# QinLab-WFU/CLIP-based-Cross-Modal-Hashing

Hardware: AMD Instinct MI355X
Metric: image+text pairs/s encoded+hashed per GPU; mAP@K eval wallclock (64-bit) (higher is better)
Workload: dtype bf16

## Files before the change

clip-based-cross-modal-hashing_amd/csrc/gemm_lc.hip:

```cpp
#include <cstdlib>
#include <cstring>

#include "cmh_common.h"

#include <hip/hip_ext.h>

namespace cmh {

typedef __attribute__((ext_vector_type(8))) __bf16 lc_bf16x8_t;
typedef __attribute__((ext_vector_type(4))) float lc_f32x4_t;
typedef __attribute__((ext_vector_type(2))) float lc_f32x2_t;
typedef __attribute__((ext_vector_type(4))) uint32_t lc_u32x4_t;
typedef __attribute__((ext_vector_type(2))) unsigned lc_u2_t;
typedef const __attribute__((address_space(1))) void* lc_gptr_t;
typedef __attribute__((address_space(3))) void* lc_lptr_t;

constexpr int lcBM = 128, lcBN = 256;
constexpr int lcRowBytes = 128;
constexpr int lcWBytes = lcBN * lcRowBytes;
constexpr int lcSTG = lcWBytes + lcBM * lcRowBytes;

struct LcProblem {
  const char* X; const char* W; const float* bias; const void* residual; void* out;
  const int* m_dev;
  int Mub, N, K;
  const float* colscale = nullptr;
  float alpha = 1.f, oscale = 1.f;
};

__device__ __forceinline__ int lc_swz(int row, int chunk) { return row * lcRowBytes + ((chunk ^ (row & 7)) << 4); }

#define LC_READ(dst, addr, off) asm volatile("ds_read_b128 %0, %1 offset:" #off : "=v"(dst) : "v"(addr))
typedef const __attribute__((address_space(3))) lc_u32x4_t* lc_lds_u4p;
__device__ __forceinline__ lc_u32x4_t lc_lds_read(uint32_t addr) { return *reinterpret_cast<lc_lds_u4p>(static_cast<size_t>(addr)); }

#ifdef LC_STAMPS
__device__ unsigned long long g_lc_stamps[256 * 8];
#define LC_T() __builtin_amdgcn_s_memtime()
#endif


template <int BM, bool GRP, int BK = 64>
struct LcSchedule {
  int M0, M1;
  int tiles_n0, tiles_n1, slot, per;
  DealShare sh0, sh1;
  int n_first, my_tiles;
  int nk0, nk1, S;
  __device__ __forceinline__ LcSchedule(const LcProblem& p0, const LcProblem& p1) {
    M0 = p0.Mub;
    if (p0.m_dev) { const int md = *p0.m_dev; M0 = md < M0 ? md : M0; }
    M0 = __builtin_amdgcn_readfirstlane(M0);
    M1 = 0;
    if constexpr (GRP) {
      M1 = p1.Mub;
      if (p1.m_dev) { const int md = *p1.m_dev; M1 = md < M1 ? md : M1; }
      M1 = __builtin_amdgcn_readfirstlane(M1);
    }
    tiles_n0 = p0.N / lcBN; tiles_n1 = GRP ? p1.N / lcBN : 1;
    const int total0 = tiles_n0 * ((M0 + BM - 1) / BM);
    const int total1 = GRP ? tiles_n1 * ((M1 + BM - 1) / BM) : 0;
    const int xcd = blockIdx.x & 7;
    slot = blockIdx.x >> 3; per = gridDim.x >> 3;
    sh0 = deal_share(total0, xcd); sh1 = deal_share(total1, xcd);
    n_first = deal_count(sh0.len, slot, per);
    my_tiles = deal_count(sh0.len + sh1.len, slot, per);
  }
  __device__ __forceinline__ void count_ksteps(const LcProblem& p0, const LcProblem& p1) {
    nk0 = p0.K / BK; nk1 = GRP ? p1.K / BK : 0;
    S = n_first * nk0 + (my_tiles - n_first) * nk1;
  }
  __device__ void tile_of(int ti, bool& second, int& m0, int& n0) const {
    second = GRP && ti >= n_first;
    const int logical = deal_tile(slot + ti * per, second, sh0, sh1);
    const int tn_cnt = second ? tiles_n1 : tiles_n0;
    const int tm = logical / tn_cnt;
    m0 = tm * BM;
    n0 = (logical - tm * tn_cnt) * lcBN;
  }
};

constexpr int lc_pieces(int bm) { return 8 + bm / 32; }
#define LC_VMCNT(n) asm volatile("s_waitcnt vmcnt(%0)" ::"n"(n) : "memory")
template <int BM, bool GRP, int ABL = 0, int LDS_BYTES>
__device__ __forceinline__ void lc_loader_wave(const LcSchedule<BM, GRP>& sc, char (&lds)[LDS_BYTES], int wid, int lane, int epi,
                                               const char* X0, const char* W0, const float* B0, int K0, const char* X1, const char* W1,
                                               const float* B1, int K1) {
  constexpr int XP = BM / 32;
  constexpr int PIECES = lc_pieces(BM);
  static_assert(2 * PIECES < 64, "the counted waits must fit gfx950's 6-bit vmcnt field");
  constexpr int STG = lcWBytes + BM * lcRowBytes;
  static_assert(LDS_BYTES == 3 * STG + 2 * 1024, "the ring of three stages, then the two bias rows");
  const int sub = lane >> 3, ch = lane & 7;
  uint32_t offW[8], offX[XP];
  const char* Wt = nullptr;
  const char* Xt = nullptr;
  const char* Bt = nullptr;
  int i_nk = 0;
  int w_prob = -1;
  auto set_tile = [&](int ti) {
    bool second; int m0, n0;
    sc.tile_of(ti, second, m0, n0);
    const uint32_t rs = static_cast<uint32_t>(second ? K1 : K0) * 2;
    if (w_prob != static_cast<int>(second)) {
      w_prob = static_cast<int>(second);
#pragma unroll
      for (int i = 0; i < 8; ++i) {
        const int row = (wid * 8 + i) * 8 + sub;
        offW[i] = static_cast<uint32_t>(row) * rs + ((ch ^ (row & 7)) << 4);
      }
    }
    i_nk = second ? sc.nk1 : sc.nk0;
    const int Mp = second ? sc.M1 : sc.M0;
    Wt = (second ? W1 : W0) + static_cast<size_t>(n0) * rs;
    Xt = second ? X1 : X0;
    Bt = reinterpret_cast<const char*>((second ? B1 : B0) + n0);
#pragma unroll
    for (int i = 0; i < XP; ++i) {
      const int row = (wid * XP + i) * 8 + sub;
      int xr = m0 + row;
      xr = xr < Mp ? xr : Mp - 1;
      offX[i] = static_cast<uint32_t>(xr) * rs + ((ch ^ (row & 7)) << 4);
    }
  };
  int i_tile = 0, i_kt = 0, ibuf = 0;
  set_tile(0);
  const bool bias_wave = wid == 0 && (epi & EPI_BIAS);
  auto issue_stage = [&]() {
    char* base = lds + ibuf * STG;
    const uint32_t koff = static_cast<uint32_t>(i_kt) * lcRowBytes;
    if (i_kt == 0 && bias_wave)
      __builtin_amdgcn_global_load_lds((lc_gptr_t)(Bt + lane * 16), (lc_lptr_t)(lds + 3 * STG + (i_tile & 1) * 1024), 16, 0, 0);
#pragma unroll
    for (int i = 0; i < 8; ++i)
      __builtin_amdgcn_global_load_lds((lc_gptr_t)(Wt + koff + offW[i]), (lc_lptr_t)(base + (wid * 8 + i) * 1024), 16, 0, 0);
#pragma unroll
    for (int i = 0; i < XP; ++i)
      __builtin_amdgcn_global_load_lds((lc_gptr_t)(Xt + koff + offX[i]), (lc_lptr_t)(base + lcWBytes + (wid * XP + i) * 1024), 16, 0, 0);
    ibuf = ibuf == 2 ? 0 : ibuf + 1;
    if (++i_kt == i_nk) {
      i_kt = 0;
      if (++i_tile < sc.my_tiles) set_tile(i_tile);
    }
  };
  const int S = sc.S;
  issue_stage();
  if (S > 1) issue_stage();
  if (S > 2) issue_stage();
  if (S > 2) LC_VMCNT(2 * PIECES);
  else if (S > 1) LC_VMCNT(PIECES);
  else LC_VMCNT(0);
  __builtin_amdgcn_s_barrier();
  for (int s = 0; s < S; ++s) {
    if (s + 2 < S && !(ABL & 4)) LC_VMCNT(PIECES);
    else LC_VMCNT(0);
    __builtin_amdgcn_s_barrier();
    if (s + 3 < S && !(ABL & 2)) issue_stage();
  }
}

__device__ __forceinline__ lc_f32x4_t lc_mfma_bf16(const lc_u32x4_t& w, const lc_u32x4_t& x, const lc_f32x4_t& cin) {
  return __builtin_amdgcn_mfma_f32_16x16x32_bf16(__builtin_bit_cast(lc_bf16x8_t, w), __builtin_bit_cast(lc_bf16x8_t, x), cin, 0, 0, 0);
}
template <int NP, int ROW0 = 0>
__device__ __forceinline__ void lc_store_parked(const lc_u32x4_t (&pend)[NP], int idx, char* base, uint32_t off0, uint32_t ldn) {
  static_assert(NP == 4 || NP == 8, "four or eight parked pieces");
  char* p = base + (off0 + static_cast<uint32_t>(ROW0 + (idx >> 1)) * 16u * ldn + static_cast<uint32_t>(idx & 1) * 64u);
  switch (idx) {
    case 0: *reinterpret_cast<lc_u32x4_t*>(p) = pend[0]; break;
    case 1: *reinterpret_cast<lc_u32x4_t*>(p) = pend[1]; break;
    case 2: *reinterpret_cast<lc_u32x4_t*>(p) = pend[2]; break;
    case 3: *reinterpret_cast<lc_u32x4_t*>(p) = pend[3]; break;
    case 4: *reinterpret_cast<lc_u32x4_t*>(p) = pend[NP > 4 ? 4 : 3]; break;
    case 5: *reinterpret_cast<lc_u32x4_t*>(p) = pend[NP > 4 ? 5 : 3]; break;
    case 6: *reinterpret_cast<lc_u32x4_t*>(p) = pend[NP > 4 ? 6 : 3]; break;
    default: *reinterpret_cast<lc_u32x4_t*>(p) = pend[NP - 1]; break;
  }
}
template <int BM, bool GRP>
__device__ __forceinline__ void lc_residual_of(const LcSchedule<BM, GRP>& sc, int ti, int wm, int wn, const void* R0, int N0,
                                               const void* R1, int N1, const uint16_t*& base, int& ld, int& rows) {
  bool second; int m0, n0;
  sc.tile_of(ti, second, m0, n0);
  ld = second ? N1 : N0;
  rows = (second ? sc.M1 : sc.M0) - (m0 + wm * (BM / 2));
  base = reinterpret_cast<const uint16_t*>(second ? R1 : R0) + static_cast<size_t>(m0 + wm * (BM / 2)) * ld + n0 + wn * 64;
}
__device__ __forceinline__ lc_u32x4_t lc_res_piece(const uint16_t* base, int ld, int rows, int frow, int fq, int b, int pr) {
  int r = b * 16 + frow;
  r = r < rows ? r : rows - 1;
  return *reinterpret_cast<const lc_u32x4_t*>(base + static_cast<size_t>(r) * ld + (fq & 1) * 16 + (fq & 2) * 4 + 32 * pr);
// ... 540 lines not shown
constexpr int lc3STG = lcWBytes + lc3BM * lcRowBytes;

template <bool GRP, int RES, bool F16O>
__global__ __launch_bounds__(768) void gemm_lc3_kernel(LcProblem p0, LcProblem p1, int epi) {
  __shared__ __attribute__((aligned(1024))) char lds[3 * lc3STG + 2 * 1024];
  const int tid = threadIdx.x;
  const int lane = tid & 63;
  const int wid = __builtin_amdgcn_readfirstlane(tid >> 6);

  const char* const X0 = p0.X; const char* const W0 = p0.W; const float* const B0 = p0.bias; void* const O0 = p0.out;
  const void* const R0 = p0.residual;
  const int N0 = p0.N, K0 = p0.K;
  const char* const X1 = p1.X; const char* const W1 = p1.W; const float* const B1 = p1.bias; void* const O1 = p1.out;
  const void* const R1 = p1.residual;
  const int N1 = p1.N, K1 = p1.K;
  int M0 = p0.Mub;
  if (p0.m_dev) { const int md = *p0.m_dev; M0 = md < M0 ? md : M0; }
  M0 = __builtin_amdgcn_readfirstlane(M0);
  int M1 = 0;
  if constexpr (GRP) {
    M1 = p1.Mub;
    if (p1.m_dev) { const int md = *p1.m_dev; M1 = md < M1 ? md : M1; }
    M1 = __builtin_amdgcn_readfirstlane(M1);
  }
  const int tiles_n0 = N0 / lcBN, tiles_n1 = GRP ? N1 / lcBN : 1;
  const int total0 = tiles_n0 * ((M0 + lc3BM - 1) / lc3BM);
  const int total1 = GRP ? tiles_n1 * ((M1 + lc3BM - 1) / lc3BM) : 0;
  const int xcd = blockIdx.x & 7, slot = blockIdx.x >> 3, per = gridDim.x >> 3;
  const int q0 = total0 >> 3, r0 = total0 & 7, q1 = total1 >> 3, r1 = total1 & 7;
  const int lo0 = xcd < r0 ? xcd * (q0 + 1) : r0 * (q0 + 1) + (xcd - r0) * q0, len0 = xcd < r0 ? q0 + 1 : q0;
  const int lo1 = xcd < r1 ? xcd * (q1 + 1) : r1 * (q1 + 1) + (xcd - r1) * q1, len1 = xcd < r1 ? q1 + 1 : q1;
  const int n_first = slot < len0 ? (len0 - slot + per - 1) / per : 0;
  const int span = len0 + len1;
  const int my_tiles = slot < span ? (span - slot + per - 1) / per : 0;
  if (my_tiles == 0) return;
  const int nk0 = K0 / 64, nk1 = GRP ? K1 / 64 : 0;
  const int S = n_first * nk0 + (my_tiles - n_first) * nk1;
  auto tile_of = [&](int ti, bool& second, int& m0, int& n0) {
    const int j = slot + ti * per;
    second = GRP && ti >= n_first;
    const int logical = second ? lo1 + (j - len0) : lo0 + j;
    const int tn_cnt = second ? tiles_n1 : tiles_n0;
    const int tm = logical / tn_cnt;
    m0 = tm * lc3BM;
    n0 = (logical - tm * tn_cnt) * lcBN;
  };

  if (wid < 4) {
    const int sub = lane >> 3, ch = lane & 7;
    uint32_t offW[8], offX[5];
    const char* Wt = nullptr;
    const char* Xt = nullptr;
    const char* Bt = nullptr;
    int i_nk = 0;
    int w_prob = -1;
    auto set_tile = [&](int ti) {
      bool second; int m0, n0;
      tile_of(ti, second, m0, n0);
      const uint32_t rs = static_cast<uint32_t>(second ? K1 : K0) * 2;
      if (w_prob != static_cast<int>(second)) {
        w_prob = static_cast<int>(second);
#pragma unroll
        for (int i = 0; i < 8; ++i) {
          const int row = (wid * 8 + i) * 8 + sub;
          offW[i] = static_cast<uint32_t>(row) * rs + ((ch ^ (row & 7)) << 4);
        }
      }
      i_nk = second ? nk1 : nk0;
      const int Mp = second ? M1 : M0;
      Wt = (second ? W1 : W0) + static_cast<size_t>(n0) * rs;
      Xt = second ? X1 : X0;
      Bt = reinterpret_cast<const char*>((second ? B1 : B0) + n0);
#pragma unroll
      for (int i = 0; i < 5; ++i) {
        const int row = (wid * 5 + i) * 8 + sub;
        int xr = m0 + row;
        xr = xr < Mp ? xr : Mp - 1;
        offX[i] = static_cast<uint32_t>(xr) * rs + ((ch ^ (row & 7)) << 4);
      }
    };
    int i_tile = 0, i_kt = 0, ibuf = 0;
    set_tile(0);
    const bool bias_wave = wid == 0 && (epi & EPI_BIAS);
    auto issue_stage = [&]() {
      char* base = lds + ibuf * lc3STG;
      const uint32_t koff = static_cast<uint32_t>(i_kt) * lcRowBytes;
      if (i_kt == 0 && bias_wave)
        __builtin_amdgcn_global_load_lds((lc_gptr_t)(Bt + lane * 16), (lc_lptr_t)(lds + 3 * lc3STG + (i_tile & 1) * 1024), 16, 0, 0);
#pragma unroll
      for (int i = 0; i < 8; ++i)
        __builtin_amdgcn_global_load_lds((lc_gptr_t)(Wt + koff + offW[i]), (lc_lptr_t)(base + (wid * 8 + i) * 1024), 16, 0, 0);
#pragma unroll
      for (int i = 0; i < 5; ++i)
        __builtin_amdgcn_global_load_lds((lc_gptr_t)(Xt + koff + offX[i]), (lc_lptr_t)(base + lcWBytes + (wid * 5 + i) * 1024), 16, 0, 0);
      ibuf = ibuf == 2 ? 0 : ibuf + 1;
      if (++i_kt == i_nk) {
        i_kt = 0;
        if (++i_tile < my_tiles) set_tile(i_tile);
      }
    };
    issue_stage();
    if (S > 1) issue_stage();
    if (S > 2) issue_stage();
    if (S > 2) LC_VMCNT(2 * lc_pieces(lc3BM));
    else if (S > 1) LC_VMCNT(lc_pieces(lc3BM));
    else LC_VMCNT(0);
    __builtin_amdgcn_s_barrier();
    for (int s = 0; s < S; ++s) {
      if (s + 2 < S) LC_VMCNT(lc_pieces(lc3BM));
      else LC_VMCNT(0);
      __builtin_amdgcn_s_barrier();
      if (s + 3 < S) issue_stage();
    }
    return;
  }

  const int c = wid - 4;
  const int wm = c >> 2, wn = c & 3;
  const int frow = lane & 15, fq = lane >> 4;
  const uint32_t lds_base = static_cast<uint32_t>(reinterpret_cast<uintptr_t>((lc_lptr_t)lds));
  const uint32_t aW = lds_base + lc_swz(wn * 64 + frow, fq);
  const uint32_t aX = lds_base + lcWBytes + lc_swz(wm * 80 + frow, fq);

  lc_f32x4_t acc[4][5];
  lc_u32x4_t fw[4], fx[5];
  lc_u32x4_t pend[8];
  int pend_idx = 8;
  char* pend_base = nullptr;
  uint32_t pend_off0 = 0, pend_ldn = 0;
  [[maybe_unused]] int res_kt = -1;
  [[maybe_unused]] const uint16_t* rq_base = nullptr;
  [[maybe_unused]] int rq_ld = 0, rq_rows = 0;

  void* out = O0;
  int N = N0, M = M0, nk = nk0;
  [[maybe_unused]] auto to_problem1 = [&]() { out = O1; N = N1; M = M1; nk = nk1; };
  if constexpr (GRP) { if (n_first == 0) to_problem1(); }

  auto store_pending = [&](int idx) __attribute__((always_inline)) {
    lc_store_parked(pend, idx, pend_base, pend_off0, pend_ldn);
  };
  [[maybe_unused]] auto residual_of = [&](int ti, const uint16_t*& base, int& ld, int& rows) __attribute__((always_inline)) {
    bool second; int m0, n0;
    tile_of(ti, second, m0, n0);
    ld = second ? N1 : N0;
    rows = (second ? M1 : M0) - (m0 + wm * 80);
    base = reinterpret_cast<const uint16_t*>(second ? R1 : R0) + static_cast<size_t>(m0 + wm * 80) * ld + n0 + wn * 64;
  };
  [[maybe_unused]] auto res_piece = [&](const uint16_t* base, int ld, int rows, int b, int pr) __attribute__((always_inline)) {
    return lc_res_piece(base, ld, rows, frow, fq, b, pr);
  };
  [[maybe_unused]] auto add_piece = [&](int b, int pr, const lc_u32x4_t& qv) __attribute__((always_inline)) { lc_add_piece(acc, b, pr, qv); };

  int cur = 0;
  if constexpr (RES == 1) {
    const uint16_t* rb; int ld, rows;
    residual_of(0, rb, ld, rows);
#pragma unroll
    for (int a = 0; a < 4; ++a)
#pragma unroll
      for (int b = 0; b < 5; ++b) acc[a][b] = lc_f32x4_t{0.f, 0.f, 0.f, 0.f};
#pragma unroll
    for (int b = 0; b < 5; ++b)
#pragma unroll
      for (int pr = 0; pr < 2; ++pr) add_piece(b, pr, res_piece(rb, ld, rows, b, pr));
  }
  __builtin_amdgcn_s_barrier();
  asm volatile("" ::: "memory");
#pragma unroll
  for (int b = 0; b < 5; ++b) fx[b] = lc_lds_read(aX + b * 2048);
#pragma unroll
  for (int a = 0; a < 4; ++a) fw[a] = lc_lds_read(aW + a * 2048);

#define L3_GROUP(a)                                                                                    \
  do {                                                                                                 \
    acc[a][0] = lc_mfma_bf16(fw[a], fx[0], acc[a][0]);                                                 \
    acc[a][1] = lc_mfma_bf16(fw[a], fx[1], acc[a][1]);                                                 \
    acc[a][2] = lc_mfma_bf16(fw[a], fx[2], acc[a][2]);                                                 \
    acc[a][3] = lc_mfma_bf16(fw[a], fx[3], acc[a][3]);                                                 \
    acc[a][4] = lc_mfma_bf16(fw[a], fx[4], acc[a][4]);                                                 \
    __builtin_amdgcn_sched_barrier(0);                                                                 \
  } while (0)
#define L3_LAST(wsrc, xsrc)                                                                            \
  do {                                                                                                 \
    acc[3][0] = lc_mfma_bf16(fw[3], fx[0], acc[3][0]);                                                 \
    __builtin_amdgcn_sched_barrier(0);                                                                 \
    fx[0] = lc_lds_read((xsrc));                                                                       \
    __builtin_amdgcn_sched_barrier(0);                                                                 \
    acc[3][1] = lc_mfma_bf16(fw[3], fx[1], acc[3][1]);                                                 \
    __builtin_amdgcn_sched_barrier(0);                                                                 \
    fx[1] = lc_lds_read((xsrc) + 2048);                                                                \
    __builtin_amdgcn_sched_barrier(0);                                                                 \
    acc[3][2] = lc_mfma_bf16(fw[3], fx[2], acc[3][2]);                                                 \
    __builtin_amdgcn_sched_barrier(0);                                                                 \
    fx[2] = lc_lds_read((xsrc) + 4096);                                                                \
    __builtin_amdgcn_sched_barrier(0);                                                                 \
    acc[3][3] = lc_mfma_bf16(fw[3], fx[3], acc[3][3]);                                                 \
    __builtin_amdgcn_sched_barrier(0);                                                                 \
    fx[3] = lc_lds_read((xsrc) + 6144);                                                                \
    __builtin_amdgcn_sched_barrier(0);                                                                 \
    acc[3][4] = lc_mfma_bf16(fw[3], fx[4], acc[3][4]);                                                 \
    __builtin_amdgcn_sched_barrier(0);                                                                 \
    fx[4] = lc_lds_read((xsrc) + 8192);                                                                \
    fw[3] = lc_lds_read((wsrc) + 6144);                                                                \
    __builtin_amdgcn_sched_barrier(0);                                                                 \
  } while (0)
#define L3_REFILL_W(a, wsrc)                                                                           \
  do {                                                                                                 \
    fw[a] = lc_lds_read((wsrc) + (a) * 2048);                                                          \
    __builtin_amdgcn_sched_barrier(0);                                                                 \
  } while (0)

  auto kstep = [&](int kt) __attribute__((always_inline)) {
    const uint32_t bo = static_cast<uint32_t>(cur) * lc3STG;
    const uint32_t w1 = (aW + bo) ^ 64u, x1 = (aX + bo) ^ 64u;
    L3_GROUP(0); L3_REFILL_W(0, w1);
    L3_GROUP(1); L3_REFILL_W(1, w1);
    if (pend_idx < 8) {
      store_pending(pend_idx); store_pending(pend_idx + 1);
      pend_idx += 2;
      asm volatile("" : "+s"(pend_idx));
      __builtin_amdgcn_sched_barrier(0);
    }
    if constexpr (RES != 0) {
      if (kt == res_kt) {
#pragma unroll
        for (int b = 0; b < 4; ++b)
#pragma unroll
          for (int pr = 0; pr < 2; ++pr) pend[2 * b + pr] = res_piece(rq_base, rq_ld, rq_rows, b, pr);
        __builtin_amdgcn_sched_barrier(0);
      }
    }
    L3_GROUP(2); L3_REFILL_W(2, w1);
    L3_LAST(w1, x1);
    const int nxt = cur == 2 ? 0 : cur + 1;
    const uint32_t bn = static_cast<uint32_t>(nxt) * lc3STG;
    const uint32_t w0 = aW + bn, x0 = aX + bn;
    L3_GROUP(0);
    L3_GROUP(1);
    __builtin_amdgcn_s_waitcnt(0xC07F);
    __builtin_amdgcn_s_barrier();
    asm volatile("" ::: "memory");
    __builtin_amdgcn_sched_barrier(0);
    L3_REFILL_W(0, w0); L3_REFILL_W(1, w0);
    L3_GROUP(2); L3_REFILL_W(2, w0);
    L3_LAST(w0, x0);
    cur = nxt;
  };

  for (int ti = 0; ti < my_tiles; ++ti) {
    bool second; int m0, n0;
    tile_of(ti, second, m0, n0);
    if constexpr (GRP) { if (ti == n_first && ti > 0) to_problem1(); }
    if constexpr (RES != 1) {
#pragma unroll
      for (int a = 0; a < 4; ++a)
#pragma unroll
        for (int b = 0; b < 5; ++b) acc[a][b] = lc_f32x4_t{0.f, 0.f, 0.f, 0.f};
    }
    if constexpr (RES == 1) { res_kt = ti + 1 < my_tiles ? 4 : -1; if (ti + 1 < my_tiles) residual_of(ti + 1, rq_base, rq_ld, rq_rows); }
    if constexpr (RES == 2) { res_kt = 4; residual_of(ti, rq_base, rq_ld, rq_rows); }
    if constexpr (RES != 0) asm volatile("" : "+s"(res_kt));
    for (int kt = 0; kt < nk; ++kt) {
      asm volatile("" : "+s"(kt));
      kstep(kt);
    }

    [[maybe_unused]] lc_u32x4_t r4[2];
    if constexpr (RES == 2) { r4[0] = res_piece(rq_base, rq_ld, rq_rows, 4, 0); r4[1] = res_piece(rq_base, rq_ld, rq_rows, 4, 1); }
    if constexpr (RES == 1) {
      if (res_kt >= 0) { r4[0] = res_piece(rq_base, rq_ld, rq_rows, 4, 0); r4[1] = res_piece(rq_base, rq_ld, rq_rows, 4, 1); }
    }
    if (epi & EPI_BIAS) {
      const uint32_t ab = lds_base + 3 * lc3STG + (ti & 1) * 1024 + (wn * 64 + fq * 4) * 4;
      lc_f32x4_t bv[4];
#pragma unroll
      for (int a = 0; a < 4; ++a) bv[a] = __builtin_bit_cast(lc_f32x4_t, lc_lds_read(ab + a * 64));
#pragma unroll
      for (int a = 0; a < 4; ++a)
#pragma unroll
        for (int b = 0; b < 5; ++b) acc[a][b] += bv[a];
    }
    if (epi & EPI_QUICKGELU) lc_quickgelu(acc);
    if constexpr (RES == 2) {
#pragma unroll
      for (int b = 0; b < 4; ++b)
#pragma unroll
        for (int pr = 0; pr < 2; ++pr) add_piece(b, pr, pend[2 * b + pr]);
      add_piece(4, 0, r4[0]); add_piece(4, 1, r4[1]);
    }
    __builtin_amdgcn_sched_barrier(0);
    {
      char* const obase = static_cast<char*>(out) + (static_cast<size_t>(m0) * N + n0) * 2;
      const uint32_t ldn = static_cast<uint32_t>(N) * 2;
      const uint32_t off0 = static_cast<uint32_t>(wm * 80 + frow) * ldn + static_cast<uint32_t>(wn * 64 + (fq & 1) * 16 + (fq & 2) * 4) * 2;
      const bool full = m0 + lc3BM <= M;
      lc_u32x4_t own4[2];
#pragma unroll
      for (int b = 0; b < 5; ++b)
#pragma unroll
        for (int pr = 0; pr < 2; ++pr) {
          const lc_u32x4_t val = lc_pack_piece<F16O>(acc, b, pr);
          if constexpr (RES == 1) {
            const lc_u32x4_t nextres = b < 4 ? pend[2 * b + pr] : r4[pr];
            acc[2 * pr][b] = lc_f32x4_t{0.f, 0.f, 0.f, 0.f};
            acc[2 * pr + 1][b] = lc_f32x4_t{0.f, 0.f, 0.f, 0.f};
            if (res_kt >= 0) add_piece(b, pr, nextres);
          }
          if (b < 4) pend[2 * b + pr] = val;
          else own4[pr] = val;
        }
      if (!(epi & 256)) {
        if (full) {
#pragma unroll
          for (int pr = 0; pr < 2; ++pr) *reinterpret_cast<lc_u32x4_t*>(obase + (off0 + 64u * ldn + pr * 64)) = own4[pr];
        } else if (m0 + wm * 80 + 64 + frow < M) {
#pragma unroll
          for (int pr = 0; pr < 2; ++pr) *reinterpret_cast<lc_u32x4_t*>(obase + (off0 + 64u * ldn + pr * 64)) = own4[pr];
        }
      }
      pend_base = obase; pend_off0 = off0; pend_ldn = ldn;
      if (full && ti + 1 < my_tiles && !(epi & 256)) {
        pend_idx = 0;
        asm volatile("" : "+s"(pend_idx));
      } else if (!(epi & 256)) {
#pragma unroll
        for (int b = 0; b < 4; ++b)
#pragma unroll
          for (int pr = 0; pr < 2; ++pr)
            if (m0 + wm * 80 + b * 16 + frow < M)
              *reinterpret_cast<lc_u32x4_t*>(obase + (off0 + static_cast<uint32_t>(b * 16) * ldn + pr * 64)) = pend[2 * b + pr];
      }
    }
  }
#undef L3_GROUP
#undef L3_LAST
#undef L3_REFILL_W
}

template <bool GRP>
__global__ __launch_bounds__(768) void gemm_lc2q_kernel(LcProblem p0, LcProblem p1, int epi) {
  static_assert(!GRP, "first form: plain launches");
  __shared__ __attribute__((aligned(1024))) char lds[3 * lcSTG];
  const int tid = threadIdx.x;
  const int lane = tid & 63;
  const int wid = __builtin_amdgcn_readfirstlane(tid >> 6);
  const char* const X0 = p0.X; const char* const W0 = p0.W; const float* const B0 = p0.bias; void* const O0 = p0.out;
  const float* const CS0 = p0.colscale; const float alpha0 = p0.alpha;
  const int N0 = p0.N, K0 = p0.K;
  LcSchedule<lcBM, false, 128> sc(p0, p1);
  if (sc.my_tiles == 0) return;
  sc.count_ksteps(p0, p1);
  const int M0 = sc.M0, nk0 = sc.nk0, my_tiles = sc.my_tiles;
  if (wid < 4) {
    const int S = sc.S;
    const int sub = lane >> 3, ch = lane & 7;
    uint32_t offW[8], offX[4];
    const char* Wt = nullptr;
    const uint32_t rs = static_cast<uint32_t>(K0);
#pragma unroll
    for (int i = 0; i < 8; ++i) {
      const int row = (wid * 8 + i) * 8 + sub;
      offW[i] = static_cast<uint32_t>(row) * rs + ((ch ^ (row & 7)) << 4);
    }
    auto set_tile = [&](int ti) {
      bool second; int m0, n0;
      sc.tile_of(ti, second, m0, n0);
      Wt = W0 + static_cast<size_t>(n0) * rs;
#pragma unroll
      for (int i = 0; i < 4; ++i) {
        const int row = (wid * 4 + i) * 8 + sub;
        int xr = m0 + row;
        xr = xr < M0 ? xr : M0 - 1;
        offX[i] = static_cast<uint32_t>(xr) * rs + ((ch ^ (row & 7)) << 4);
      }
    };
    int i_tile = 0, i_kt = 0, ibuf = 0;
    set_tile(0);
    auto issue_stage = [&]() {
      char* base = lds + ibuf * lcSTG;
      const uint32_t koff = static_cast<uint32_t>(i_kt) * lcRowBytes;
#pragma unroll
      for (int i = 0; i < 8; ++i)
        __builtin_amdgcn_global_load_lds((lc_gptr_t)(Wt + koff + offW[i]), (lc_lptr_t)(base + (wid * 8 + i) * 1024), 16, 0, 0);
#pragma unroll
      for (int i = 0; i < 4; ++i)
        __builtin_amdgcn_global_load_lds((lc_gptr_t)(X0 + koff + offX[i]), (lc_lptr_t)(base + lcWBytes + (wid * 4 + i) * 1024), 16, 0, 0);
      ibuf = ibuf == 2 ? 0 : ibuf + 1;
      if (++i_kt == nk0) {
        i_kt = 0;
        if (++i_tile < my_tiles) set_tile(i_tile);
      }
    };
    issue_stage();
    if (S > 1) issue_stage();
    if (S > 2) issue_stage();
    if (S > 2) LC_VMCNT(2 * lc_pieces(lcBM));
    else if (S > 1) LC_VMCNT(lc_pieces(lcBM));
    else LC_VMCNT(0);
    __builtin_amdgcn_s_barrier();
    for (int s = 0; s < S; ++s) {
      if (s + 2 < S) LC_VMCNT(lc_pieces(lcBM));
      else LC_VMCNT(0);
      __builtin_amdgcn_s_barrier();
      if (s + 3 < S) issue_stage();
    }
    return;
  }
  const int c = wid - 4;
  const int wm = c >> 2, wn = c & 3;
  const int frow = lane & 15, fq = lane >> 4;
  const uint32_t lds_base = static_cast<uint32_t>(reinterpret_cast<uintptr_t>((lc_lptr_t)lds));
  const uint32_t aW = lds_base + lc_swz(wn * 64 + frow, fq);
  const uint32_t aX = lds_base + lcWBytes + lc_swz(wm * 64 + frow, fq);
  typedef __attribute__((ext_vector_type(8))) int lc_i32x8_t;
  lc_f32x4_t acc[4][4];
  lc_u32x4_t fw[4][2], fx[4][2];
  lc_u32x4_t pend[4];
  int pend_idx = 4;
  char* pend_base = nullptr;
  uint32_t pend_off0 = 0, pend_ldn = 0;
  auto store_pending = [&](int idx) __attribute__((always_inline)) {
    lc_store_parked<4, 2>(pend, idx, pend_base, pend_off0, pend_ldn);
  };
  auto mfma8 = [&](int a, int b) __attribute__((always_inline)) {
    lc_i32x8_t va, vb;
#pragma unroll
    for (int j = 0; j < 4; ++j) {
      va[j] = static_cast<int>(fw[a][0][j]); va[4 + j] = static_cast<int>(fw[a][1][j]);
      vb[j] = static_cast<int>(fx[b][0][j]); vb[4 + j] = static_cast<int>(fx[b][1][j]);
    }
    acc[a][b] = __builtin_amdgcn_mfma_scale_f32_16x16x128_f8f6f4(va, vb, acc[a][b], 0, 0, 0, 0x7f7f7f7f, 0, 0x7f7f7f7f);
  };
#define Q_READ2(dst, addr, off)                                                                                   \
  do {                                                                                                            \
    asm volatile("ds_read_b128 %0, %1 offset:%2" : "=v"(dst[0]) : "v"(addr), "n"(off));                          \
    asm volatile("ds_read_b128 %0, %1 offset:%2" : "=v"(dst[1]) : "v"((addr) ^ 64u), "n"(off));                  \
  } while (0)
#define Q_WAIT_ALL()                                                                                               \
  asm volatile("s_waitcnt lgkmcnt(0)"                                                                             \
               : "+v"(fw[0][0]), "+v"(fw[0][1]), "+v"(fw[1][0]), "+v"(fw[1][1]), "+v"(fw[2][0]), "+v"(fw[2][1]), "+v"(fw[3][0]), "+v"(fw[3][1]), \
                 "+v"(fx[0][0]), "+v"(fx[0][1]), "+v"(fx[1][0]), "+v"(fx[1][1]), "+v"(fx[2][0]), "+v"(fx[2][1]), "+v"(fx[3][0]), "+v"(fx[3][1])::"memory")
  int cur = 0;
  __builtin_amdgcn_s_barrier();
  Q_READ2(fx[0], aX, 0); Q_READ2(fx[1], aX, 2048); Q_READ2(fx[2], aX, 4096); Q_READ2(fx[3], aX, 6144);
  Q_READ2(fw[0], aW, 0); Q_READ2(fw[1], aW, 2048); Q_READ2(fw[2], aW, 4096); Q_READ2(fw[3], aW, 6144);
  auto kstep = [&]() __attribute__((always_inline)) {
    Q_WAIT_ALL();
    __builtin_amdgcn_s_barrier();
    __builtin_amdgcn_sched_barrier(0);
    const int nxt = cur == 2 ? 0 : cur + 1;
    const uint32_t bn = static_cast<uint32_t>(nxt) * lcSTG;
    const uint32_t w0 = aW + bn, x0 = aX + bn;
    mfma8(0, 0); mfma8(0, 1); mfma8(0, 2); mfma8(0, 3);
    __builtin_amdgcn_sched_barrier(0);
    Q_READ2(fw[0], w0, 0);
    __builtin_amdgcn_sched_barrier(0);
    mfma8(1, 0); mfma8(1, 1); mfma8(1, 2); mfma8(1, 3);
    __builtin_amdgcn_sched_barrier(0);
    if (pend_idx < 4) {
      store_pending(pend_idx); store_pending(pend_idx + 1);
      pend_idx += 2;
      asm volatile("" : "+s"(pend_idx));
      __builtin_amdgcn_sched_barrier(0);
    }
    Q_READ2(fw[1], w0, 2048);
    __builtin_amdgcn_sched_barrier(0);
    mfma8(2, 0); mfma8(2, 1); mfma8(2, 2); mfma8(2, 3);
    __builtin_amdgcn_sched_barrier(0);
    Q_READ2(fw[2], w0, 4096);
    __builtin_amdgcn_sched_barrier(0);
    mfma8(3, 0);
    __builtin_amdgcn_sched_barrier(0);
    Q_READ2(fx[0], x0, 0);
    __builtin_amdgcn_sched_barrier(0);
    mfma8(3, 1);
    __builtin_amdgcn_sched_barrier(0);
    Q_READ2(fx[1], x0, 2048);
    __builtin_amdgcn_sched_barrier(0);
    mfma8(3, 2);
    __builtin_amdgcn_sched_barrier(0);
    Q_READ2(fx[2], x0, 4096);
    __builtin_amdgcn_sched_barrier(0);
    mfma8(3, 3);
    __builtin_amdgcn_sched_barrier(0);
    Q_READ2(fx[3], x0, 6144);
    Q_READ2(fw[3], w0, 6144);
    __builtin_amdgcn_sched_barrier(0);
    cur = nxt;
  };
  for (int ti = 0; ti < my_tiles; ++ti) {
    bool second; int m0, n0;
    sc.tile_of(ti, second, m0, n0);
    lc_zero(acc);
    for (int kt = 0; kt < nk0; ++kt) kstep();
#pragma unroll
    for (int a = 0; a < 4; ++a) {
      const lc_f32x4_t cs = *reinterpret_cast<const lc_f32x4_t*>(CS0 + n0 + wn * 64 + a * 16 + fq * 4) * alpha0;
      const lc_f32x4_t bv = (epi & EPI_BIAS) ? *reinterpret_cast<const lc_f32x4_t*>(B0 + n0 + wn * 64 + a * 16 + fq * 4) : lc_f32x4_t{0.f, 0.f, 0.f, 0.f};
#pragma unroll
      for (int b = 0; b < 4; ++b) acc[a][b] = acc[a][b] * cs + bv;
    }
    char* const obase = static_cast<char*>(O0) + (static_cast<size_t>(m0) * N0 + n0) * 2;
    const uint32_t ldn = static_cast<uint32_t>(N0) * 2;
    const uint32_t off0 = static_cast<uint32_t>(wm * 64 + frow) * ldn + static_cast<uint32_t>(wn * 64 + (fq & 1) * 16 + (fq & 2) * 4) * 2;
    const bool park = m0 + lcBM <= M0 && ti + 1 < my_tiles && !(epi & 256);
#pragma unroll
    for (int b = 0; b < 4; ++b)
#pragma unroll
      for (int pr = 0; pr < 2; ++pr) {
        const lc_u32x4_t val = lc_pack_piece<false>(acc, b, pr);
        if (b >= 2) pend[(b - 2) * 2 + pr] = val;
        if ((b < 2 || !park) && m0 + wm * 64 + b * 16 + frow < M0 && !(epi & 256))
          *reinterpret_cast<lc_u32x4_t*>(obase + (off0 + static_cast<uint32_t>(b * 16) * ldn + pr * 64)) = val;
      }
    if (park) {
      pend_base = obase; pend_off0 = off0; pend_ldn = ldn;
      pend_idx = 0;
      asm volatile("" : "+s"(pend_idx));
    }
  }
  asm volatile("s_waitcnt lgkmcnt(0)" ::: "memory");
#undef Q_READ2
#undef Q_WAIT_ALL
}

int launch_gemm_lc2q(const GemmProblem& g, int epi, const GemmPlan& p, hipStream_t st, hipEvent_t ev0, hipEvent_t ev1) {
  LcProblem P0{static_cast<const char*>(g.A), static_cast<const char*>(g.W), g.bias, g.residual, g.out, g.m_dev, g.M, g.N, g.K};
  P0.colscale = g.colscale; P0.alpha = g.alpha; P0.oscale = g.oscale;
  const LcProblem P1{};
  if (ev0) hipExtLaunchKernelGGL((gemm_lc2q_kernel<false>), dim3(p.grid), dim3(768), 0, st, ev0, ev1, 0, P0, P1, epi);
  else hipLaunchKernelGGL((gemm_lc2q_kernel<false>), dim3(p.grid), dim3(768), 0, st, P0, P1, epi);
  CMH_CHECK_LAUNCH("gemm (lc2q)");
  return 0;
}
bool gemm_lc2q_takes(int N, int K, int epi) {
  return gemm_lc_mode() == 7 && N % lcBN == 0 && K % 128 == 0 && K >= 512 &&
         (epi & ~(EPI_BIAS | EPI_SCALE | 256)) == EPI_OUT_BF16;
}

static int lc_env_mode() { static const int m = []() { const char* e = getenv("CMH_GEMM_LC"); return e ? atoi(e) : 8; }(); return m; }
static int g_lc_mode = -1;
int gemm_lc_mode() { return g_lc_mode < 0 ? lc_env_mode() : g_lc_mode; }
void gemm_lc_set_mode(int m) { g_lc_mode = m; }

bool gemm_lc_takes(int dt, int N, int K, int epi) {
  if (dt != CMH_BF16 || N % lcBN != 0 || K % 64 != 0 || K < 256) return false;
  if (gemm_lc_mode() >= 4) {
    if (K < 512) return false;
  }
  if (!(epi & (EPI_OUT_BF16 | EPI_OUT_F16)) || ((epi & EPI_OUT_BF16) && (epi & EPI_OUT_F16))) return false;
  if (epi & ~(EPI_BIAS | EPI_QUICKGELU | EPI_RESIDUAL | EPI_RES_F16 | EPI_OUT_BF16 | EPI_OUT_F16 | 256)) return false;
  if ((epi & EPI_RESIDUAL) && !((epi & EPI_RES_F16) && (epi & EPI_OUT_F16))) return false;
  if ((epi & EPI_RESIDUAL) && (epi & EPI_QUICKGELU)) return false;
  return true;
}

int launch_gemm_lc(const GemmProblem& a, const GemmProblem* b, int epi, const GemmPlan& p, hipStream_t st, hipEvent_t ev0, hipEvent_t ev1) {
  auto prob = [](const GemmProblem& g) {
    return LcProblem{static_cast<const char*>(g.A), static_cast<const char*>(g.W), g.bias, g.residual, g.out, g.m_dev, g.M, g.N, g.K};
  };
  const int grid = p.grid, res = p.res;
  const bool f16 = (epi & EPI_OUT_F16) != 0;
  const LcProblem P0 = prob(a), P1 = b ? prob(*b) : LcProblem{};
#define LC_GO(KERNEL, THREADS, ...)                                                                                           \
  do {                                                                                                                       \
    if (ev0) hipExtLaunchKernelGGL((KERNEL<__VA_ARGS__>), dim3(grid), dim3(THREADS), 0, st, ev0, ev1, 0, P0, P1, epi);       \
    else hipLaunchKernelGGL((KERNEL<__VA_ARGS__>), dim3(grid), dim3(THREADS), 0, st, P0, P1, epi);                           \
  } while (0)
#define LC_GO_G(KERNEL, THREADS, G)                                                                                           \
  do {                                                                                                                       \
    if (res == 1) LC_GO(KERNEL, THREADS, G, 1, true);                                                                        \
    else if (res == 2) LC_GO(KERNEL, THREADS, G, 2, true);                                                                   \
    else if (f16) LC_GO(KERNEL, THREADS, G, 0, true);                                                                        \
    else LC_GO(KERNEL, THREADS, G, 0, false);                                                                                \
  } while (0)
#define LC_GO_ALL(KERNEL, THREADS) do { if (b) LC_GO_G(KERNEL, THREADS, true); else LC_GO_G(KERNEL, THREADS, false); } while (0)
  static const int abl = []() { const char* e = getenv("CMH_LC_ABL"); return e ? atoi(e) : 0; }();
  if (p.family == GEMM_LC3) {
    LC_GO_ALL(gemm_lc3_kernel, 768);
    CMH_CHECK_LAUNCH("gemm (lc3)");
  } else if (p.family == GEMM_LC2) {
    LC_GO_ALL(gemm_lc2_kernel, 768);
    CMH_CHECK_LAUNCH("gemm (lc2)");
  } else if (abl && !b && res != 1 && !f16) {
    if (abl == 1) LC_GO(gemm_lc_kernel, 512, false, 0, false, 1);
    else if (abl == 2) LC_GO(gemm_lc_kernel, 512, false, 0, false, 2);
    else if (abl == 3) LC_GO(gemm_lc_kernel, 512, false, 0, false, 3);
    else LC_GO(gemm_lc_kernel, 512, false, 0, false, 4);
    CMH_CHECK_LAUNCH("gemm (lc, diagnostic)");
  } else {
    LC_GO_ALL(gemm_lc_kernel, 512);
    CMH_CHECK_LAUNCH("gemm (lc)");
  }
#undef LC_GO_ALL
#undef LC_GO_G
#undef LC_GO
  return 0;
}

}

#ifdef LC_STAMPS
extern "C" int cmh_debug_lc_stamps(unsigned long long* host_out) {
  return hipMemcpyFromSymbol(host_out, HIP_SYMBOL(cmh::g_lc_stamps), sizeof(unsigned long long) * 256 * 8) == hipSuccess ? 0 : -1;
}
#endif

extern "C" int cmh_set_gemm_lc(int32_t mode) {
  CMH_CHECK_ARG(mode >= -1 && mode <= 9 && mode != 5 && mode != 6, "set_gemm_lc: mode %d (-1 environment, 0 the wide kernel only, 1 / 2 / 3 the 8-wave kernel for every eligible launch - 2: all but QuickGELU launches, 4 the 12-wave 128-row form for every block launch, 7 fp8 QKV, 8 per launch the 12-wave 160-row form or the wide kernel, by cost (default), 9 the 12-wave 160-row form for every block launch)", mode);
  cmh::gemm_lc_set_mode(mode);
  return CMH_OK;
}
```

Before: 68490.

## Add LC3 GEMM variant interleaving parked QuickGELU epilogue into next tile's MFMAs

Adds a specialized gemm_lc3g kernel for bias+QuickGELU outputs without residual. The first NPARK epilogue pieces of each full tile are parked in registers, then their QuickGELU, packing and stores are spread across the MFMA issue slots of the next tile's first k-steps, so the epilogue overlaps with matrix compute. It is enabled by default (opt out with CMH_LC3_DGE=0). It also adds optional timestamp instrumentation under LC_STAMPS. This raises register pressure and makes scheduling more complex.

Measured after the change: 69460 (median of 6 runs). 1.01x the previous value.

```diff
diff --git a/clip-based-cross-modal-hashing_amd/csrc/gemm_lc.hip b/clip-based-cross-modal-hashing_amd/csrc/gemm_lc.hip
--- a/clip-based-cross-modal-hashing_amd/csrc/gemm_lc.hip
+++ b/clip-based-cross-modal-hashing_amd/csrc/gemm_lc.hip
@@ -37,6 +37,22 @@
 #ifdef LC_STAMPS
 __device__ unsigned long long g_lc_stamps[256 * 8];
 #define LC_T() __builtin_amdgcn_s_memtime()
+#define LC3_ST_BEGIN() const unsigned long long st_t0 = LC_T(), st_r0 = __builtin_amdgcn_s_memrealtime(); unsigned long long st_first = 0, st_k = 0, st_e = 0, st_g = 0, st_mark = 0
+#define LC3_ST_FIRST() do { st_mark = LC_T(); st_first = st_mark - st_t0; } while (0)
+#define LC3_ST_LAP(sum) do { const unsigned long long t_ = LC_T(); sum += t_ - st_mark; st_mark = t_; } while (0)
+#define LC3_ST_END(S_, TILES_)                                                                                              \
+  do {                                                                                                                      \
+    if (c == 0 && lane == 0 && blockIdx.x < 256) {                                                                          \
+      unsigned long long* o = g_lc_stamps + blockIdx.x * 8;                                                                 \
+      o[0] = LC_T() - st_t0; o[1] = __builtin_amdgcn_s_memrealtime() - st_r0; o[2] = st_first; o[3] = st_k; o[4] = st_e;    \
+      o[5] = static_cast<unsigned long long>(S_); o[6] = static_cast<unsigned long long>(TILES_); o[7] = st_g;              \
+    }                                                                                                                       \
+  } while (0)
+#else
+#define LC3_ST_BEGIN() do {} while (0)
+#define LC3_ST_FIRST() do {} while (0)
+#define LC3_ST_LAP(sum) do {} while (0)
+#define LC3_ST_END(S_, TILES_) do {} while (0)
 #endif
 
 
@@ -883,6 +899,7 @@
   };
   [[maybe_unused]] auto add_piece = [&](int b, int pr, const lc_u32x4_t& qv) __attribute__((always_inline)) { lc_add_piece(acc, b, pr, qv); };
 
+  LC3_ST_BEGIN();
   int cur = 0;
   if constexpr (RES == 1) {
     const uint16_t* rb; int ld, rows;
@@ -898,6 +915,7 @@
   }
   __builtin_amdgcn_s_barrier();
   asm volatile("" ::: "memory");
+  LC3_ST_FIRST();
 #pragma unroll
   for (int b = 0; b < 5; ++b) fx[b] = lc_lds_read(aX + b * 2048);
 #pragma unroll
@@ -992,10 +1010,12 @@
     if constexpr (RES == 1) { res_kt = ti + 1 < my_tiles ? 4 : -1; if (ti + 1 < my_tiles) residual_of(ti + 1, rq_base, rq_ld, rq_rows); }
     if constexpr (RES == 2) { res_kt = 4; residual_of(ti, rq_base, rq_ld, rq_rows); }
     if constexpr (RES != 0) asm volatile("" : "+s"(res_kt));
+    LC3_ST_LAP(st_g);
     for (int kt = 0; kt < nk; ++kt) {
       asm volatile("" : "+s"(kt));
       kstep(kt);
     }
+    LC3_ST_LAP(st_k);
 
     [[maybe_unused]] lc_u32x4_t r4[2];
     if constexpr (RES == 2) { r4[0] = res_piece(rq_base, rq_ld, rq_rows, 4, 0); r4[1] = res_piece(rq_base, rq_ld, rq_rows, 4, 1); }
@@ -1063,10 +1083,240 @@
               *reinterpret_cast<lc_u32x4_t*>(obase + (off0 + static_cast<uint32_t>(b * 16) * ldn + pr * 64)) = pend[2 * b + pr];
       }
     }
-  }
+    LC3_ST_LAP(st_e);
+  }
+  LC3_ST_END(S, my_tiles);
 #undef L3_GROUP
 #undef L3_LAST
 #undef L3_REFILL_W
+}
+
+template <int MF>
+__device__ __forceinline__ void lc_quickgelu_piece(lc_f32x4_t (&acc)[4][MF], int b, int pr) {
+#pragma unroll
+  for (int a = 2 * pr; a < 2 * pr + 2; ++a)
+#pragma unroll
+    for (int j = 0; j < 4; j += 2) {
+      const lc_f32x2_t v = {acc[a][b][j], acc[a][b][j + 1]};
+      const lc_f32x2_t t = v * lc_f32x2_t{-2.4554669595930157f, -2.4554669595930157f};
+      const lc_f32x2_t d = lc_f32x2_t{__builtin_amdgcn_exp2f(t[0]), __builtin_amdgcn_exp2f(t[1])} + lc_f32x2_t{1.0f, 1.0f};
+      const lc_f32x2_t o = v * lc_f32x2_t{__builtin_amdgcn_rcpf(d[0]), __builtin_amdgcn_rcpf(d[1])};
+      acc[a][b][j] = o[0];
+      acc[a][b][j + 1] = o[1];
+    }
+}
+
+template <bool GRP, bool F16O, int NPARK = 3>
+__global__ __launch_bounds__(768) void gemm_lc3g_kernel(LcProblem p0, LcProblem p1, int epi) {
+  __shared__ __attribute__((aligned(1024))) char lds[3 * lc3STG + 2 * 1024];
+  const int tid = threadIdx.x;
+  const int lane = tid & 63;
+  const int wid = __builtin_amdgcn_readfirstlane(tid >> 6);
+
+  const char* const X0 = p0.X; const char* const W0 = p0.W; const float* const B0 = p0.bias; void* const O0 = p0.out;
+  const int N0 = p0.N, K0 = p0.K;
+  const char* const X1 = p1.X; const char* const W1 = p1.W; const float* const B1 = p1.bias; void* const O1 = p1.out;
+  const int N1 = p1.N, K1 = p1.K;
+  LcSchedule<lc3BM, GRP> sc(p0, p1);
+  if (sc.my_tiles == 0) return;
+  sc.count_ksteps(p0, p1);
+  const int n_first = sc.n_first, my_tiles = sc.my_tiles;
+
+  if (wid < 4) {
+    lc_loader_wave<lc3BM, GRP>(sc, lds, wid, lane, epi, X0, W0, B0, K0, X1, W1, B1, K1);
+    return;
+  }
+
+  const int c = wid - 4;
+  const int wm = c >> 2, wn = c & 3;
+  const int frow = lane & 15, fq = lane >> 4;
+  const uint32_t lds_base = static_cast<uint32_t>(reinterpret_cast<uintptr_t>((lc_lptr_t)lds));
+  const uint32_t aW = lds_base + lc_swz(wn * 64 + frow, fq);
+  const uint32_t aX = lds_base + lcWBytes + lc_swz(wm * 80 + frow, fq);
+
+  lc_f32x4_t acc[4][5];
+  lc_u32x4_t fw[4], fx[5];
+  lc_f32x4_t park[4][2];
+  bool parked = false;
+  char* pend_base = nullptr;
+  uint32_t pend_ldn = 0;
+
+  void* out = O0;
+  int N = N0, M = sc.M0, nk = sc.nk0;
+  [[maybe_unused]] auto to_problem1 = [&]() { out = O1; N = N1; M = sc.M1; nk = sc.nk1; };
+  if constexpr (GRP) { if (n_first == 0) to_problem1(); }
+
+  LC3_ST_BEGIN();
+  int cur = 0;
+  __builtin_amdgcn_s_barrier();
+  asm volatile("" ::: "memory");
+  LC3_ST_FIRST();
+#pragma unroll
+  for (int b = 0; b < 5; ++b) fx[b] = lc_lds_read(aX + b * 2048);
+#pragma unroll
+  for (int a = 0; a < 4; ++a) fw[a] = lc_lds_read(aW + a * 2048);
+
+  struct Piece { float g0, g1; };
+  auto micro = [&](auto jc, Piece& pc, auto sc_) __attribute__((always_inline)) {
+    constexpr int J = decltype(jc)::value;
+    constexpr int s = decltype(sc_)::value;
+    if constexpr (J >= 0) {
+      constexpr int PB = J >> 1, PR = J & 1;
+      lc_f32x4_t& A = park[2 * PR][PB];
+      if constexpr (s < 32) {
+        constexpr int q = s >> 3;
+        const lc_f32x4_t& src = q < 2 ? A : park[2 * PR + 1][PB];
+        const float v0 = src[2 * (q & 1)], v1 = src[2 * (q & 1) + 1];
+        switch (s & 7) {
+          case 0: pc.g0 = v0 * -2.4554669595930157f; break;
+          case 1: pc.g0 = __builtin_amdgcn_exp2f(pc.g0); break;
+          case 2: pc.g1 = v1 * -2.4554669595930157f; pc.g0 = pc.g0 + 1.0f; break;
+          case 3: pc.g1 = __builtin_amdgcn_exp2f(pc.g1); break;
+          case 4: pc.g0 = __builtin_amdgcn_rcpf(pc.g0); break;
+          case 5: pc.g1 = pc.g1 + 1.0f; pc.g0 = v0 * pc.g0; break;
+          case 6: pc.g1 = __builtin_amdgcn_rcpf(pc.g1); break;
+          default:
+            pc.g1 = v1 * pc.g1;
+            A[q] = __builtin_bit_cast(float, F16O ? pack_f16x2(pc.g0, pc.g1) : pack_bf16x2(pc.g0, pc.g1));
+            break;
+        }
+        __builtin_amdgcn_sched_barrier(0);
+      } else if constexpr (s == 33) {
+        const float w0 = A[0], w1 = A[1], w2 = A[2], w3 = A[3];
+        const lc_u2_t s0 = __builtin_amdgcn_permlane16_swap(__builtin_bit_cast(uint32_t, w0), __builtin_bit_cast(uint32_t, w2), false, false);
+        const lc_u2_t s1 = __builtin_amdgcn_permlane16_swap(__builtin_bit_cast(uint32_t, w1), __builtin_bit_cast(uint32_t, w3), false, false);
+        int ln = static_cast<int>(__builtin_amdgcn_mbcnt_hi(~0u, __builtin_amdgcn_mbcnt_lo(~0u, 0u)));
+        asm volatile("" : "+v"(ln));
+        const uint32_t po = static_cast<uint32_t>(wm * 80 + PB * 16 + (ln & 15)) * pend_ldn +
+                            static_cast<uint32_t>(wn * 64 + ((ln >> 4) & 1) * 16 + ((ln >> 4) & 2) * 4) * 2 + PR * 64;
+        *reinterpret_cast<lc_u32x4_t*>(pend_base + po) = lc_u32x4_t{s0[0], s1[0], s0[1], s1[1]};
+        __builtin_amdgcn_sched_barrier(0);
+      }
+    }
+  };
+
+#define G3_MFMA(jc, a, b, S0)                                                                          \
+  do {                                                                                                 \
+    acc[a][b] = lc_mfma_bf16(fw[a], fx[b], acc[a][b]);                                                 \
+    micro(jc, pc, std::integral_constant<int, (S0) + 5 * (a) + (b)>{});                                                                   \
+  } while (0)
+#define G3_GROUP(jc, a, S0)                                                                            \
+  do {                                                                                                 \
+    G3_MFMA(jc, a, 0, S0); G3_MFMA(jc, a, 1, S0); G3_MFMA(jc, a, 2, S0); G3_MFMA(jc, a, 3, S0); G3_MFMA(jc, a, 4, S0); \
+    __builtin_amdgcn_sched_barrier(0);                                                                 \
+  } while (0)
+#define G3_LAST(jc, S0, wsrc, xsrc)                                                                    \
+  do {                                                                                                 \
+    G3_MFMA(jc, 3, 0, S0);                                                                             \
+    __builtin_amdgcn_sched_barrier(0);                                                                 \
+    fx[0] = lc_lds_read((xsrc));                                                                       \
+    __builtin_amdgcn_sched_barrier(0);                                                                 \
+    G3_MFMA(jc, 3, 1, S0);                                                                             \
+    __builtin_amdgcn_sched_barrier(0);                                                                 \
+    fx[1] = lc_lds_read((xsrc) + 2048);                                                                \
+    __builtin_amdgcn_sched_barrier(0);                                                                 \
+    G3_MFMA(jc, 3, 2, S0);                                                                             \
+    __builtin_amdgcn_sched_barrier(0);                                                                 \
+    fx[2] = lc_lds_read((xsrc) + 4096);                                                                \
+    __builtin_amdgcn_sched_barrier(0);                                                                 \
+    G3_MFMA(jc, 3, 3, S0);                                                                             \
+    __builtin_amdgcn_sched_barrier(0);                                                                 \
+    fx[3] = lc_lds_read((xsrc) + 6144);                                                                \
+    __builtin_amdgcn_sched_barrier(0);                                                                 \
+    G3_MFMA(jc, 3, 4, S0);                                                                             \
+    __builtin_amdgcn_sched_barrier(0);                                                                 \
+    fx[4] = lc_lds_read((xsrc) + 8192);                                                                \
+    fw[3] = lc_lds_read((wsrc) + 6144);                                                                \
+    __builtin_amdgcn_sched_barrier(0);                                                                 \
+  } while (0)
+#define G3_REFILL_W(a, wsrc)                                                                           \
+  do {                                                                                                 \
+    fw[a] = lc_lds_read((wsrc) + (a) * 2048);                                                          \
+    __builtin_amdgcn_sched_barrier(0);                                                                 \
+  } while (0)
+
+  auto kstep = [&](auto jc) __attribute__((always_inline)) {
+    [[maybe_unused]] Piece pc;
+    const uint32_t bo = static_cast<uint32_t>(cur) * lc3STG;
+    const uint32_t w1 = (aW + bo) ^ 64u, x1 = (aX + bo) ^ 64u;
+    G3_GROUP(jc, 0, 0); G3_REFILL_W(0, w1);
+    G3_GROUP(jc, 1, 0); G3_REFILL_W(1, w1);
+    G3_GROUP(jc, 2, 0); G3_REFILL_W(2, w1);
+    G3_LAST(jc, 0, w1, x1);
+    const int nxt = cur == 2 ? 0 : cur + 1;
+    const uint32_t bn = static_cast<uint32_t>(nxt) * lc3STG;
+    const uint32_t w0 = aW + bn, x0 = aX + bn;
+    G3_GROUP(jc, 0, 20);
+    G3_GROUP(jc, 1, 20);
+    __builtin_amdgcn_s_waitcnt(0xC07F);
+    __builtin_amdgcn_s_barrier();
+    asm volatile("" ::: "memory");
+    __builtin_amdgcn_sched_barrier(0);
+    G3_REFILL_W(0, w0); G3_REFILL_W(1, w0);
+    G3_GROUP(jc, 2, 20); G3_REFILL_W(2, w0);
+    G3_LAST(jc, 20, w0, x0);
+    cur = nxt;
+  };
+
+  for (int ti = 0; ti < my_tiles; ++ti) {
+    bool second; int m0, n0;
+    sc.tile_of(ti, second, m0, n0);
+    if constexpr (GRP) { if (ti == n_first && ti > 0) to_problem1(); }
+#pragma unroll
+    for (int a = 0; a < 4; ++a)
+#pragma unroll
+      for (int b = 0; b < 5; ++b) acc[a][b] = lc_f32x4_t{0.f, 0.f, 0.f, 0.f};
+#pragma unroll
+    for (int a = 0; a < 4; ++a)
+#pragma unroll
+      for (int b = 0; b < 5; ++b) asm volatile("" : "+v"(acc[a][b]));
+    LC3_ST_LAP(st_g);
+    int kt = 0;
+    if (parked) {
+      kstep(std::integral_constant<int, 0>{});
+      if constexpr (NPARK > 1) kstep(std::integral_constant<int, 1>{});
+      if constexpr (NPARK > 2) kstep(std::integral_constant<int, 2>{});
+      if constexpr (NPARK > 3) kstep(std::integral_constant<int, 3>{});
+      kt = NPARK;
+    }
+    for (; kt < nk; ++kt) {
+      asm volatile("" : "+s"(kt));
+      kstep(std::integral_constant<int, -1>{});
+    }
+    LC3_ST_LAP(st_k);
+
+    int lane_e = static_cast<int>(__builtin_amdgcn_mbcnt_hi(~0u, __builtin_amdgcn_mbcnt_lo(~0u, 0u)));
+    asm volatile("" : "+v"(lane_e));
+    const int frow_e = lane_e & 15, fq_e = lane_e >> 4;
+    lc_add_bias(acc, lds_base + 3 * lc3STG + (ti & 1) * 1024 + (wn * 64 + fq_e * 4) * 4);
+    __builtin_amdgcn_sched_barrier(0);
+    char* const obase = static_cast<char*>(out) + (static_cast<size_t>(m0) * N + n0) * 2;
+    const uint32_t ldn = static_cast<uint32_t>(N) * 2;
+    const uint32_t off0 = static_cast<uint32_t>(wm * 80 + frow_e) * ldn + static_cast<uint32_t>(wn * 64 + (fq_e & 1) * 16 + (fq_e & 2) * 4) * 2;
+    const bool full = m0 + lc3BM <= M;
+    parked = full && ti + 1 < my_tiles && !(epi & 256);
+    if (parked) { pend_base = obase; pend_ldn = ldn; }
+#pragma unroll
+    for (int b = 0; b < 5; ++b)
+#pragma unroll
+      for (int pr = 0; pr < 2; ++pr) {
+        if (2 * b + pr < NPARK) {
+          park[2 * pr][b < 2 ? b : 0] = acc[2 * pr][b]; park[2 * pr + 1][b < 2 ? b : 0] = acc[2 * pr + 1][b];
+          if (parked) continue;
+        }
+        __builtin_amdgcn_sched_barrier(0);
+        lc_quickgelu_piece(acc, b, pr);
+        const lc_u32x4_t val = lc_pack_piece<F16O>(acc, b, pr);
+        if (full && !(epi & 256)) *reinterpret_cast<lc_u32x4_t*>(obase + (off0 + static_cast<uint32_t>(b * 16) * ldn + pr * 64)) = val;
+        else if (m0 + wm * 80 + b * 16 + frow_e < M && !(epi & 256)) *reinterpret_cast<lc_u32x4_t*>(obase + (off0 + static_cast<uint32_t>(b * 16) * ldn + pr * 64)) = val;
+      }
+    LC3_ST_LAP(st_e);
+  }
+  LC3_ST_END(sc.S, my_tiles);
+#undef G3_MFMA
+#undef G3_GROUP
+#undef G3_LAST
+#undef G3_REFILL_W
 }
 
 template <bool GRP>
@@ -1274,6 +1524,7 @@
 static int g_lc_mode = -1;
 int gemm_lc_mode() { return g_lc_mode < 0 ? lc_env_mode() : g_lc_mode; }
 void gemm_lc_set_mode(int m) { g_lc_mode = m; }
+static bool lc3_dge_enabled() { const char* e = getenv("CMH_LC3_DGE"); return !(e && e[0] == '0' && e[1] == 0); }
 
 bool gemm_lc_takes(int dt, int N, int K, int epi) {
   if (dt != CMH_BF16 || N % lcBN != 0 || K % 64 != 0 || K < 256) return false;
@@ -1308,7 +1559,11 @@
   } while (0)
 #define LC_GO_ALL(KERNEL, THREADS) do { if (b) LC_GO_G(KERNEL, THREADS, true); else LC_GO_G(KERNEL, THREADS, false); } while (0)
   static const int abl = []() { const char* e = getenv("CMH_LC_ABL"); return e ? atoi(e) : 0; }();
-  if (p.family == GEMM_LC3) {
+  if (p.family == GEMM_LC3 && res == 0 && (epi & EPI_BIAS) && (epi & EPI_QUICKGELU) && lc3_dge_enabled()) {
+    if (b) { if (f16) LC_GO(gemm_lc3g_kernel, 768, true, true); else LC_GO(gemm_lc3g_kernel, 768, true, false); }
+    else { if (f16) LC_GO(gemm_lc3g_kernel, 768, false, true); else LC_GO(gemm_lc3g_kernel, 768, false, false); }
+    CMH_CHECK_LAUNCH("gemm (lc3g)");
+  } else if (p.family == GEMM_LC3) {
     LC_GO_ALL(gemm_lc3_kernel, 768);
     CMH_CHECK_LAUNCH("gemm (lc3)");
   } else if (p.family == GEMM_LC2) {
```
